# ipilter/RayTracerTest

Measured on AMD Instinct MI355X. Metric: Mray/s at 1920x1080x16spp, higher is better.
Workload: dtype f32

## Files before the change

raytracertest_amd/csrc/rt_kernels.hip:

```cpp
#include <stdlib.h>

#include "rt_dense.hpp"
#include "rt_query.hpp"
#include "rt_bvh.hpp"

namespace rtk {

template <bool FMA>
__global__ __launch_bounds__(256) void prep_triangles_kernel(const float4* __restrict__ verts, uint32_t n, bool edges,
                                                              float4* __restrict__ tri_a,
                                                              float* __restrict__ tri_b,
                                                              float4* __restrict__ color,
                                                              float4* __restrict__ normals) {
  const uint32_t i = blockIdx.x * 256u + threadIdx.x;
  if (i >= n) return;
  const float4 a = verts[3 * i + 0], b = verts[3 * i + 1], c = verts[3 * i + 2];
  const V3 v0 = {a.x, a.y, a.z};
  const V3 e1 = edges ? V3{b.x, b.y, b.z} : rtd::sub({b.x, b.y, b.z}, v0);
  const V3 e2 = edges ? V3{c.x, c.y, c.z} : rtd::sub({c.x, c.y, c.z}, v0);
  tri_a[2 * i + 0] = make_float4(e2.x, e2.y, e2.z, e1.x);
  tri_a[2 * i + 1] = make_float4(e1.y, e1.z, v0.x, v0.y);
  tri_b[i] = v0.z;
  const V3 nn = Math<FMA>::normalize(Math<FMA>::cross(e1, e2));
  color[i] = make_float4(rtd::absf(nn.x), rtd::absf(nn.y), rtd::absf(nn.z), 0.0f);
  if (normals != nullptr) {
    const V3 n0 = rtd::unpack_normal(a.w), n1 = rtd::unpack_normal(b.w), n2 = rtd::unpack_normal(c.w);
    normals[3 * i + 0] = make_float4(n0.x, n0.y, n0.z, 0.0f);
    normals[3 * i + 1] = make_float4(n1.x, n1.y, n1.z, 0.0f);
    normals[3 * i + 2] = make_float4(n2.x, n2.y, n2.z, 0.0f);
  }
}

__global__ __launch_bounds__(256) void convert_kernel(const float4* __restrict__ render,
                                                       const uint32_t* __restrict__ counts,
                                                       uint32_t* __restrict__ image, uint32_t npix) {
  const uint32_t i = blockIdx.x * 256u + threadIdx.x;
  if (i >= npix) return;
  const float4 s = render[i];
  const float cnt = static_cast<float>(counts[i]);
  image[i] = rtd::pack_color(255.0f * (s.x / cnt), 255.0f * (s.y / cnt), 255.0f * (s.z / cnt));
}

template <bool FMA>
__global__ void dbg_hit_triangle_kernel(uint32_t n, const float* __restrict__ rays,
                                        const float* __restrict__ tris, int eps_mode,
                                        int* __restrict__ hit, float* __restrict__ tuv,
                                        float* __restrict__ normal, float* __restrict__ point) {
  using M = Math<FMA>;
  const uint32_t i = blockIdx.x * blockDim.x + threadIdx.x;
  if (i >= n) return;
  const float* r = rays + 6 * static_cast<size_t>(i);
  const float* q = tris + 9 * static_cast<size_t>(i);
  const V3 o = {r[0], r[1], r[2]};
  const V3 d = M::normalize({r[3], r[4], r[5]});
  const V3 a = {q[0], q[1], q[2]}, b = {q[3], q[4], q[5]}, c = {q[6], q[7], q[8]};
  const V3 e1 = rtd::sub(b, a), e2 = rtd::sub(c, a);
  float t = 0.0f, u = 0.0f, v = 0.0f;
  int stage;
  const bool h = hit_triangle_exact<FMA>(o, d, a, e1, e2, eps_mode ? FLT_EPSILON : 0.0000000001f, t, u, v, stage);
  hit[i] = h ? 1 : 0;
  tuv[3 * i + 0] = t; tuv[3 * i + 1] = u; tuv[3 * i + 2] = v;
  const V3 nn = M::normalize(M::cross(e1, e2));
// ... 256 lines not shown
      case variant(P::Classify, 2): return launch_trace_kernel<F, 2, P::Classify>(p, filter, grid, lds, st);
      case variant(P::Classify, 4): return launch_trace_kernel<F, 4, P::Classify>(p, filter, grid, lds, st);
      case variant(P::ClassifyForms, 1): return launch_trace_kernel<F, 1, P::ClassifyForms>(p, filter, grid, lds, st);
      case variant(P::ClassifyForms, 2): return launch_trace_kernel<F, 2, P::ClassifyForms>(p, filter, grid, lds, st);
      case variant(P::ClassifyForms, 4): return launch_trace_kernel<F, 4, P::ClassifyForms>(p, filter, grid, lds, st);
      case variant(P::DenseLists, 1): return launch_trace_kernel<F, 1, P::DenseLists>(p, filter, grid, lds, st);
      case variant(P::DenseLists, 2): return launch_trace_kernel<F, 2, P::DenseLists>(p, filter, grid, lds, st);
      case variant(P::DenseLists, 4): return launch_trace_kernel<F, 4, P::DenseLists>(p, filter, grid, lds, st);
    }
  };
  if (fma) launch(std::true_type{}); else launch(std::false_type{});
  return hipGetLastError();
}

int trace_occupancy(int K, size_t lds) {
  int n = 0;
  hipError_t e;
  if (K == 1) e = hipOccupancyMaxActiveBlocksPerMultiprocessor(&n, trace_kernel<true, 1, true, false, TracePath::SmallLists>, 256, lds);
  else if (K == 2) e = hipOccupancyMaxActiveBlocksPerMultiprocessor(&n, trace_kernel<true, 2, true, false, TracePath::SmallLists>, 256, lds);
  else e = hipOccupancyMaxActiveBlocksPerMultiprocessor(&n, trace_kernel<true, 4, true, false, TracePath::Classify>, 256, lds);
  return e == hipSuccess ? n : -1;
}

hipError_t launch_convert(const float4* render, const uint32_t* counts, uint32_t* image, uint32_t npix,
                          hipStream_t st) {
  if (npix == 0) return hipSuccess;
  hipLaunchKernelGGL(convert_kernel, dim3(cdiv(npix, 256)), dim3(256), 0, st, render, counts, image, npix);
  return hipGetLastError();
}

hipError_t launch_dbg_hit_triangle(bool fma, uint32_t n, const float* rays, const float* tris, int eps_mode,
                                   int* hit, float* tuv, float* normal, float* point, hipStream_t st) {
  if (n == 0) return hipSuccess;
  if (fma) hipLaunchKernelGGL(dbg_hit_triangle_kernel<true>, dim3(cdiv(n, 64)), dim3(64), 0, st, n, rays, tris, eps_mode, hit, tuv, normal, point);
  else hipLaunchKernelGGL(dbg_hit_triangle_kernel<false>, dim3(cdiv(n, 64)), dim3(64), 0, st, n, rays, tris, eps_mode, hit, tuv, normal, point);
  return hipGetLastError();
}

hipError_t launch_super_bin(const TraceParams& p, bool fma, hipStream_t st) {
  if (p.super_lists == nullptr || p.macro_bounds == nullptr || p.macro_lists == nullptr || p.n_tris == 0u || p.rows == 0u || p.W == 0u || p.super_f == 0u ||
      p.super_chunks != cdiv(p.n_tris, kSuperChunk) || p.super_chunks > kSuperMaxChunks) return hipErrorInvalidValue;
  const dim3 mgrid(cdiv(p.W, p.macro_w), cdiv(p.rows, p.macro_h));
  const dim3 sgrid(p.super_nx * cdiv(mgrid.y, p.super_f), p.super_chunks);
  if (fma) {
    hipLaunchKernelGGL(macro_bounds_kernel<true>, mgrid, dim3(256), 0, st, p);
    hipLaunchKernelGGL(super_bin_kernel<true>, sgrid, dim3(256), 0, st, p);
  } else {
    hipLaunchKernelGGL(macro_bounds_kernel<false>, mgrid, dim3(256), 0, st, p);
    hipLaunchKernelGGL(super_bin_kernel<false>, sgrid, dim3(256), 0, st, p);
  }
// ... 160 lines not shown
```

raytracertest_amd/csrc/rt_kernels.hpp:

```cpp
#pragma once
#include <hip/hip_runtime.h>
#include <stdint.h>

namespace rtk {

constexpr uint32_t kSuperChunk = 1024u, kSuperMaxChunks = 64u;

struct TraceParams {
  float4*   render;
  uint32_t* counts;
  uint32_t* rng;
  uint32_t  W, H;
  uint32_t  row0, rows;
  uint32_t  npix;
  uint32_t  samples;
  float     cam[12];
  float     half_height, aspect, focal, aperture;
  float     tile_curv, tile_round;
  const float4* tri_a;
  const float*  tri_b;
  const float4* tri_color;
  uint32_t  n_tris;
  const float4* spheres;
  uint32_t  n_spheres;
  uint32_t  chunk;
  uint32_t  bin_list;
  uint32_t  block_list;
  unsigned long long* stats;
  uint32_t* image;
  const float4* tri_n;
#ifdef RT_TIMELINE
  unsigned long long* timeline;
#endif
  uint32_t* image_host;
// ... 15 lines not shown
};

constexpr uint32_t TRACE_ZERO_ACC = 1u;
constexpr uint32_t TRACE_EMIT_IMAGE = 2u;
constexpr uint32_t TRACE_NEAREST_HIT = 4u;
constexpr uint32_t TRACE_PRETEST = 32u;
constexpr uint32_t TRACE_NO_SURE_HIT = 64u;

enum class TracePath : uint32_t {
  FullScan,
  SmallLists,
  Classify,
  ClassifyForms,
  DenseLists,
};

hipError_t launch_rng_init(uint32_t* rng, uint32_t npix, uint32_t p0, const uint32_t seeded[6],
                           const uint32_t* jump, const uint32_t* win, hipStream_t st);
hipError_t launch_prep_triangles(bool fma, bool edges, const float4* verts, uint32_t n, float4* tri_a, float* tri_b,
                                 float4* color, float4* normals, hipStream_t st);
uint32_t trace_lds_bytes(const TraceParams& p, TracePath path);
hipError_t launch_trace(const TraceParams& p, bool fma, bool filter, TracePath path, int K, hipStream_t st);
int trace_occupancy(int K, size_t lds);
hipError_t launch_convert(const float4* render, const uint32_t* counts, uint32_t* image, uint32_t npix,
                          hipStream_t st);

uint32_t query_lds_bytes(uint32_t n_tris, int K);
hipError_t launch_query(const TraceParams& p, bool fma, int K, uint32_t n, const float* rays, const uint32_t* pixels,
                        float* rays_out, float4* hits, hipStream_t st);

#define RT_BVH_RHO 0.00390625f

struct BvhParams {
  const float4* nodes;
  const float4* records;
  uint32_t n_nodes;
  uint32_t n_leaf_records;
  uint32_t n_always;
  uint32_t stack_cap;
  float rho;
};
uint32_t query_bvh_lds_bytes(uint32_t stack_cap);
hipError_t launch_query_bvh(const TraceParams& p, const BvhParams& b, bool fma, uint32_t n, const float* rays, const uint32_t* pixels,
                            float* rays_out, float4* hits, hipStream_t st);

hipError_t launch_dbg_hit_triangle(bool fma, uint32_t n, const float* rays, const float* tris, int eps_mode,
                                   int* hit, float* tuv, float* normal, float* point, hipStream_t st);
bool trace_can_fuse(TracePath path, bool filter);
// ... 19 lines not shown
```

raytracertest_amd/csrc/rt_multi_api.hpp:

```cpp
#pragma once

namespace rtr {

bool env_on(const char* name) { const char* e = getenv(name); return e && e[0] == '1'; }

void multi_push_camera(rt_tracer* t) {
  Camera c;
  { std::lock_guard<std::mutex> lk(t->state_mu); c = t->cam; }
  for (rt_tracer* b : t->mg->bands) { std::lock_guard<std::mutex> lk(b->state_mu); b->cam = c; }
}

void multi_sync_all(rt_tracer* t) {
  MultiState& m = *t->mg;
  for (rt_tracer* b : m.bands) {
    b->use_device();
    b->sync_all();
  }
  m.group.sync();
}

void multi_frame_to_host(rt_tracer* t, int b) {
  MultiState& m = *t->mg;
  Group& g = m.group;
  HIP_CHECK(hipSetDevice(g.local[0].device));
// ... 367 lines not shown
    s += "]";
  }
  s += "}";
  return s;
}

void multi_read_buffer(rt_tracer* t, int which, void* dst, size_t bytes) {
  MultiState& m = *t->mg;
  Group& g = m.group;
  multi_sync_all(t);
  if (which == RT_BUF_IMAGE || which == RT_BUF_FRAME) {
    HIP_CHECK(hipSetDevice(g.local[0].device));
    HIP_CHECK(hipMemcpy(dst, g.d_frame[g.last_b < 0 ? 0 : g.last_b], bytes, hipMemcpyDeviceToHost));
    return;
  }
  const size_t per_px = which == RT_BUF_RENDER ? sizeof(float4) : sizeof(uint32_t);
  const size_t planes = which == RT_BUF_RNG ? 6u : 1u;
  const size_t frame_px = static_cast<size_t>(t->W) * t->H;
  if (bytes < frame_px * per_px * planes) throw HipFail{"rt_tracer_read_buffer: a multi-device tracer reads whole buffers only"};
  for (size_t k = 0; k < m.bands.size(); ++k) {
    rt_tracer* band = m.bands[k];
    band->use_device();
    const size_t band_px = band->npix(), off_px = static_cast<size_t>(g.bands[k].row0) * t->W;
    for (size_t p = 0; p < planes; ++p)
      HIP_CHECK(hipMemcpy(static_cast<char*>(dst) + (p * frame_px + off_px) * per_px,
                          static_cast<const char*>(buffer_ptr(band, which)) + p * band_px * per_px, band_px * per_px,
                          hipMemcpyDeviceToHost));
  }
}

void member_join(rt_tracer* t, uint32_t n_ranks, uint32_t rank, const uint8_t id[RT_GROUP_ID_BYTES], const uint32_t* begins) {
  if (t->grp) throw HipFail{"rt_tracer_join_group: already a member of a group"};
  uint32_t r0 = 0, rn = 0;
  if (begins) {
    if (begins[0] != 0u || begins[n_ranks] != t->H) throw HipFail{"rt_tracer_join_group_bands: the bands must cover rows 0 .. full_height"};
    for (uint32_t k = 0; k < n_ranks; ++k) if (begins[k + 1] <= begins[k]) throw HipFail{"rt_tracer_join_group_bands: empty or descending band"};
    r0 = begins[rank]; rn = begins[rank + 1] - begins[rank];
  } else {
    band_rows(t->H, n_ranks, rank, r0, rn);
  }
  if (!t->band_mode && n_ranks > 1u) throw HipFail{"rt_tracer_join_group: the tracer must own a row band (rt_options.full_height)"};
  if (r0 != t->row0 || rn != t->rows)
    throw HipFail{fmt("rt_tracer_join_group: rank %u of %u owns rows [%u, %u) of %u, the tracer has [%u, %u)", rank, n_ranks, r0,
                      r0 + rn, t->H, t->row0, t->row0 + t->rows)};
  Group* g = new Group();
  g->W = t->W; g->H = t->H;
// ... 50 lines not shown
```

raytracertest_amd/csrc/rt_rng_init.hip:

```cpp
#include "rt_device_math.hpp"
#include "rt_kernels.hpp"

namespace rtk {

using rtd::Rng;

static inline uint32_t cdiv(uint32_t a, uint32_t b) { return (a + b - 1) / b; }

constexpr uint32_t kRngWinEntries = 6u * 40u * 16u;
constexpr uint32_t kRngInitThreads = 512;

__device__ __forceinline__ uint32_t wave_xor(uint32_t v) {
#pragma unroll
  for (int off = 32; off >= 1; off >>= 1) v ^= static_cast<uint32_t>(__shfl_xor(static_cast<int>(v), off, 64));
  return v;
}

__global__ __launch_bounds__(kRngInitThreads, 4) void rng_init_kernel(uint32_t* __restrict__ rng, uint32_t npix,
                                                                    uint32_t p0, Rng seeded,
                                                                    const uint32_t* __restrict__ jump,
                                                                    const uint32_t* __restrict__ win) {
  extern __shared__ uint4 s_win[];
  uint32_t* const s_w4 = reinterpret_cast<uint32_t*>(s_win + kRngWinEntries);
  for (uint32_t i = threadIdx.x; i < kRngWinEntries; i += kRngInitThreads) {
// ... 55 lines not shown
    }
    uint32_t v[5] = {u[0], u[1], u[2], u[3], u[4]};
    for (uint32_t m = 0; m < 6u; ++m) {
      const uint4* __restrict__ T = s_win + m * 640u;
      const uint32_t* __restrict__ T4 = s_w4 + m * 640u;
      uint32_t r0 = 0u, r1 = 0u, r2 = 0u, r3 = 0u, r4 = 0u;
#pragma unroll 1
      for (uint32_t w = 0; w < 5u; ++w) {
        const uint32_t vw = w == 0u ? v[0] : w == 1u ? v[1] : w == 2u ? v[2] : w == 3u ? v[3] : v[4];
        const uint4* __restrict__ Tw = T + w * 128u;
        const uint32_t* __restrict__ T4w = T4 + w * 128u;
#pragma unroll
        for (uint32_t q = 0; q < 8u; ++q) {
          const uint32_t n = (vw >> (q * 4u)) & 15u;
          const uint4 e = Tw[q * 16u + n];
          r0 ^= e.x; r1 ^= e.y; r2 ^= e.z; r3 ^= e.w;
          r4 ^= T4w[q * 16u + n];
        }
      }
      if ((lane >> m) & 1u) { v[0] = r0; v[1] = r1; v[2] = r2; v[3] = r3; v[4] = r4; }
    }
    const uint32_t i = base + lane;
    if (i < npix) {
      rng[0 * static_cast<size_t>(npix) + i] = seeded.d;
      rng[1 * static_cast<size_t>(npix) + i] = v[0];
      rng[2 * static_cast<size_t>(npix) + i] = v[1];
      rng[3 * static_cast<size_t>(npix) + i] = v[2];
      rng[4 * static_cast<size_t>(npix) + i] = v[3];
      rng[5 * static_cast<size_t>(npix) + i] = v[4];
    }
  }
}

hipError_t launch_rng_init(uint32_t* rng, uint32_t npix, uint32_t p0, const uint32_t seeded[6],
                           const uint32_t* jump, const uint32_t* win, hipStream_t st) {
  Rng s = {seeded[0], seeded[1], seeded[2], seeded[3], seeded[4], seeded[5]};
  if (npix == 0) return hipSuccess;
  const uint32_t want = cdiv(npix, kRngInitThreads);
  uint32_t blocks = 1u;
  while (blocks < 512u && blocks * 2u <= want) blocks *= 2u;
  hipLaunchKernelGGL(rng_init_kernel, dim3(blocks), dim3(kRngInitThreads), kRngWinEntries * 20u, st, rng, npix, p0, s, jump, win);
  return hipGetLastError();
}

}
```

raytracertest_amd/csrc/rt_trace.hpp:

```cpp
#pragma once
#include "rt_lists.hpp"

namespace rtk {


template <bool FMA, int K, bool FILTER, bool STATS, class GetB>
__device__ __forceinline__ void test_triangle(const float4 A0, const float4 A1, GetB get_v0z, int tri_index,
                                              const V3 (&o)[K], const V3 (&d)[K], float (&best_t)[K],
                                              int (&best_i)[K], bool nearest, bool counted_lane, uint32_t valid_k,
                                              unsigned long long (&st_exit)[4],
                                              unsigned long long (&st_skip)[4]) {
  using M = Math<FMA>;
  const V3 e2 = {A0.x, A0.y, A0.z}, e1 = {A0.w, A1.x, A1.y};

  if constexpr (!FILTER) {
    const V3 v0 = {A1.z, A1.w, get_v0z()};
#pragma unroll
    for (int k = 0; k < K; ++k) {
      float t = 0.0f, u = 0.0f, v = 0.0f;
      int stage;
      const bool h = hit_triangle_exact<FMA>(o[k], d[k], v0, e1, e2, RT_EPS, t, u, v, stage);
      if (h && (nearest ? (t > 0.0f && t < best_t[k]) : best_t[k] < t)) {
        best_t[k] = t;
        best_i[k] = tri_index;
// ... 87 lines not shown
  const uint32_t cxp = inside ? px : 0u, cyp = inside ? ly : 0u;
  const size_t pix = static_cast<size_t>(cxp) + static_cast<size_t>(cyp) * p.W;

#ifdef RT_TIMELINE
  const size_t tl_slot = ((static_cast<size_t>(by) * gxb + bx) * 4u + wave) * 16u;
  auto tl_mark = [&](uint32_t i) {
    __builtin_amdgcn_sched_barrier(0);
    if (p.timeline != nullptr && lane == 0u) p.timeline[tl_slot + i] = __builtin_amdgcn_s_memrealtime();
    __builtin_amdgcn_sched_barrier(0);
  };
  if (p.timeline != nullptr && lane == 0u) {
    uint32_t hw, xcc;
    asm volatile("s_getreg_b32 %0, hwreg(HW_REG_HW_ID)" : "=s"(hw));
    asm volatile("s_getreg_b32 %0, hwreg(HW_REG_XCC_ID)" : "=s"(xcc));
    p.timeline[tl_slot + 6] = hw;
    p.timeline[tl_slot + 7] = (static_cast<unsigned long long>(xcc) << 32) | (__builtin_amdgcn_s_memrealtime() & 0xffffffffull);
  }
  tl_mark(0);
#else
  auto tl_mark = [](uint32_t) {};
#endif
  Rng rng;
  auto load_rng = [&] {
    rng.d = p.rng[0 * static_cast<size_t>(p.npix) + pix];
    rng.v0 = p.rng[1 * static_cast<size_t>(p.npix) + pix];
    rng.v1 = p.rng[2 * static_cast<size_t>(p.npix) + pix];
    rng.v2 = p.rng[3 * static_cast<size_t>(p.npix) + pix];
    rng.v3 = p.rng[4 * static_cast<size_t>(p.npix) + pix];
    rng.v4 = p.rng[5 * static_cast<size_t>(p.npix) + pix];
  };
  constexpr bool FORMS = Path == TracePath::ClassifyForms || Path == TracePath::DenseLists;
  constexpr bool RNG_LATE = FORMS;
  constexpr bool THIRD_BLOCK = true, THIRD_WAVE = !FORMS;
  if constexpr (!RNG_LATE) load_rng();


  const bool sure_ok = Path == TracePath::SmallLists && (p.flags & (TRACE_NEAREST_HIT | TRACE_NO_SURE_HIT)) == 0u && p.n_spheres == 0u && p.tri_n == nullptr;
  bool loaded_sure = false;
  uint32_t list_word = 0u;
  if constexpr (Path == TracePath::SmallLists) {
    if (p.tile_lists != nullptr) {
      const size_t slot0 = (static_cast<size_t>(by) * gxb + bx) * 4u + wave;
      list_word = static_cast<uint32_t>(__builtin_amdgcn_readfirstlane(static_cast<int>(p.tile_lists[slot0 * (1u + p.bin_list)])));
      loaded_sure = sure_ok && (list_word >> 31) != 0u;
    }
  }
  V3 po = {0.0f, 0.0f, 0.0f}, pd = {0.0f, 0.0f, 0.0f}, focal = {0.0f, 0.0f, 0.0f};
// ... 205 lines not shown
    __builtin_amdgcn_wave_barrier();
    list_count = count;
    if constexpr (STATS) { st_bin[0] += count; st_bin[1] += 1; }
    list_complete = true;
  }
  bool forms_ready = false;
  if constexpr (Path == TracePath::ClassifyForms) {
    const uint32_t next0 = classify(0u, std::true_type{});
    list_complete = next0 >= src_count;
    forms_ready = pretest && list_complete;
  }
  if constexpr (Path == TracePath::DenseLists) forms_ready = true;
  if constexpr (RNG_LATE) load_rng();
  tl_mark(1);
  float4 sure_col = make_float4(0.0f, 0.0f, 0.0f, 0.0f);
  const bool sure_sums = Path == TracePath::SmallLists && p.sure_table != nullptr;
  if constexpr (Path == TracePath::SmallLists) { if (sure_hit_tile) sure_col = sure_sums ? p.sure_table[sure_winner] : p.tri_color[sure_winner]; }
  if constexpr (STATS && Path == TracePath::SmallLists) {
    if (lane == 0u && p.stats != nullptr)
      atomicAdd(p.stats + (sure_hit_tile ? 13 : list_count == 0u ? 11 : list_count == 1u ? 12 : list_count == 2u ? 14 : 15), 1ull);
  }
  const uint32_t iters = FUSE ? p.iters : 1u;
  float rx = 0.0f, ry = 0.0f, rz = 0.0f, rw = 0.0f;
  uint32_t cnt_first = 0u;
  for (uint32_t it = 0; it < iters; ++it) {
  if constexpr (FUSE) { ax = 0.0f; ay = 0.0f; az = 0.0f; }
  uint32_t traced_samples = p.samples;
  if constexpr (Path == TracePath::SmallLists) {
    if (sure_hit_tile) {
      rtd::rng_discard(rng, 3u * p.samples);
      if (sure_sums) { ax = sure_col.x; ay = sure_col.y; az = sure_col.z; }
      else for (uint32_t s = 0; s < p.samples; ++s) { ax += sure_col.x; ay += sure_col.y; az += sure_col.z; }
      if constexpr (STATS) st_pre += (p.samples + static_cast<uint32_t>(K) - 1u) / static_cast<uint32_t>(K);
      traced_samples = 0u;
    }
  }
  for (uint32_t s0 = 0; s0 < traced_samples; s0 += K) {
    if (s0 == static_cast<uint32_t>(K)) tl_mark(2);
    const uint32_t valid_k = (p.samples - s0 < static_cast<uint32_t>(K)) ? p.samples - s0 : static_cast<uint32_t>(K);
    V3 o[K], d[K];
    float best_t[K];
    int best_i[K];
#pragma unroll
    for (int k = 0; k < K; ++k) {
      if (static_cast<uint32_t>(k) < valid_k) get_ray<FMA>(p, focal, rng, o[k], d[k]);
      else { o[k] = {0.0f, 0.0f, 0.0f}; d[k] = {0.0f, 0.0f, -1.0f}; }
      best_t[k] = nearest ? FLT_MAX : -FLT_MAX;
// ... 147 lines not shown
            const V3 nn = M::normalize(rtd::sub(hp, {sph.x, sph.y, sph.z}));
            r = rtd::absf(nn.x); g = rtd::absf(nn.y); b = rtd::absf(nn.z);
          }
        } else {
          if constexpr (FMA) {
            r = __builtin_fmaf(d[k].x, 0.2f, 0.15f * 0.8f);
            g = __builtin_fmaf(d[k].y, 0.2f, 0.11f * 0.8f);
            b = __builtin_fmaf(d[k].z, 0.2f, 0.13f * 0.8f);
          } else {
            r = 0.15f * 0.8f + d[k].x * 0.2f;
            g = 0.11f * 0.8f + d[k].y * 0.2f;
            b = 0.13f * 0.8f + d[k].z * 0.2f;
          }
        }
        ax += r; ay += g; az += b;
      }
    }
  }

  if constexpr (FUSE) {
    if (it == 0u && !(p.flags & TRACE_ZERO_ACC) && inside) {
      const float4 r0 = p.render[pix];
      rx = r0.x; ry = r0.y; rz = r0.z; rw = r0.w;
      cnt_first = p.counts[pix];
    }
    rx += ax; ry += ay; rz += az;
  }
  }
  tl_mark(3);
  uint32_t pix_lo = static_cast<uint32_t>(pix);
  asm volatile("" : "+v"(pix_lo));
  const size_t pix_e = pix_lo;
  if (inside) {
    float4 acc_in = make_float4(0.0f, 0.0f, 0.0f, 0.0f);
    uint32_t cnt_in = 0u;
    if constexpr (!FUSE) {
      if (!(p.flags & TRACE_ZERO_ACC)) {
        acc_in = p.render[pix_e];
        cnt_in = p.counts[pix_e];
      }
    }
    const uint32_t cnt = FUSE ? cnt_first + iters * p.samples : cnt_in + p.samples;
    p.counts[pix_e] = cnt;
    float4 acc = acc_in;
    if constexpr (FUSE) {
      acc = make_float4(rx, ry, rz, rw);
    } else {
      acc.x += ax; acc.y += ay; acc.z += az;
    }
    p.render[pix_e] = acc;
    if (p.flags & TRACE_EMIT_IMAGE) {
      const float c = static_cast<float>(cnt);
      uint32_t bgra;
      if (!FUSE && sure_sums && sure_hit_tile && (p.flags & TRACE_ZERO_ACC)) bgra = __builtin_bit_cast(uint32_t, sure_col.w);
      else bgra = rtd::pack_color(255.0f * (acc.x / c), 255.0f * (acc.y / c), 255.0f * (acc.z / c));
      p.image[pix_e] = bgra;
      if (p.image_host != nullptr) p.image_host[pix_e] = bgra;
    }
    p.rng[0 * static_cast<size_t>(p.npix) + pix_e] = rng.d;
    p.rng[1 * static_cast<size_t>(p.npix) + pix_e] = rng.v0;
    p.rng[2 * static_cast<size_t>(p.npix) + pix_e] = rng.v1;
    p.rng[3 * static_cast<size_t>(p.npix) + pix_e] = rng.v2;
    p.rng[4 * static_cast<size_t>(p.npix) + pix_e] = rng.v3;
    p.rng[5 * static_cast<size_t>(p.npix) + pix_e] = rng.v4;
  }
  tl_mark(4);
  if constexpr (STATS) {
    if (lane == 0 && p.stats != nullptr) {
#pragma unroll
      for (int e = 0; e < 4; ++e) {
        atomicAdd(p.stats + e, st_exit[e]);
        atomicAdd(p.stats + 4 + e, st_skip[e]);
      }
      atomicAdd(p.stats + 8, st_bin[0]);
      atomicAdd(p.stats + 9, st_bin[1]);
      atomicAdd(p.stats + 10, st_pre);
    }
  }
}


}
// ... 1 lines not shown
```

raytracertest_amd/csrc/rt_tracer.hip:

```cpp
#include "rt_tracer.hpp"

#include <map>

namespace rtr {

std::mutex g_err_mu;
std::string g_last_error;

void set_global_error(const std::string& s) {
  std::lock_guard<std::mutex> lk(g_err_mu);
  g_last_error = s;
  static const bool log = getenv("RT_MI355X_LOG") != nullptr;
  if (log) fprintf(stderr, "[rt_mi355x] %s\n", s.c_str());
}

std::mutex g_jump_mu;
std::vector<uint32_t> g_jump_host;
std::map<int, uint32_t*> g_jump_dev;

const std::vector<uint32_t>& jump_host() {
  std::lock_guard<std::mutex> lk(g_jump_mu);
  if (g_jump_host.empty()) g_jump_host = rth::build_jump_table();
  return g_jump_host;
}
// ... 484 lines not shown
    t->launch_instrumented(p, samples);
    HIP_CHECK(hipMemcpy(out, counters.get(), 16 * sizeof(uint64_t), hipMemcpyDeviceToHost));
  });
}

int rt_tracer_sync(rt_tracer* t) {
  if (!t) return RT_ERR_INVALID;
  if (t->mg) return guarded(t, [&] { multi_sync_all(t); });
  return guarded(t, [&] {
    t->use_device();
    t->sync_all();
    if (t->grp) t->grp->sync();
  });
}

int rt_tracer_kernel_time(rt_tracer* t, double* total_ms, uint64_t* launches, int reset_after) {
  return read_clock(t, false, total_ms, launches, reset_after);
}
int rt_tracer_launch_time(rt_tracer* t, double* total_ms, uint64_t* launches, int reset_after) {
  return read_clock(t, true, total_ms, launches, reset_after);
}

size_t rt_tracer_buffer_bytes(rt_tracer* t, int which) { return t ? buffer_bytes(t, which) : 0; }
void* rt_tracer_device_pointer(rt_tracer* t, int which) { return t ? buffer_ptr(t, which) : nullptr; }

int rt_tracer_read_buffer(rt_tracer* t, int which, void* dst, size_t bytes) {
  if (!t || !dst) return RT_ERR_INVALID;
  if (t->mg) {
    if (bytes > buffer_bytes(t, which) || buffer_bytes(t, which) == 0) return RT_ERR_INVALID;
    return guarded(t, [&] { multi_read_buffer(t, which, dst, bytes); });
  }
  if (buffer_ptr(t, which) == nullptr || bytes > buffer_bytes(t, which)) return RT_ERR_INVALID;
  return guarded(t, [&] {
    t->use_device();
    HIP_CHECK(hipStreamSynchronize(t->main_stream()));
    if (t->grp) t->grp->sync();
    HIP_CHECK(hipMemcpy(dst, buffer_ptr(t, which), bytes, hipMemcpyDeviceToHost));
  });
}

int rt_tracer_copy_buffer_to_device(rt_tracer* t, int which, void* dst_device, size_t bytes) {
  if (!t || !dst_device || buffer_ptr(t, which) == nullptr || bytes > buffer_bytes(t, which)) return RT_ERR_INVALID;
  if (t->mg) return guarded(t, [&] {
    multi_sync_all(t);
    HIP_CHECK(hipSetDevice(t->mg->group.local[0].device));
    HIP_CHECK(hipMemcpy(dst_device, buffer_ptr(t, which), bytes, hipMemcpyDeviceToDevice));
  });
  return guarded(t, [&] {
    t->use_device();
    if (t->grp && which == RT_BUF_FRAME) t->grp->sync();
    HIP_CHECK(hipMemcpyAsync(dst_device, buffer_ptr(t, which), bytes, hipMemcpyDeviceToDevice, t->main_stream()));
    HIP_CHECK(hipStreamSynchronize(t->main_stream()));
  });
}

int rt_tracer_copy_buffer_to_device_async(rt_tracer* t, int which, void* dst_device, size_t bytes) {
  if (!t || !dst_device || buffer_ptr(t, which) == nullptr || bytes > buffer_bytes(t, which)) return RT_ERR_INVALID;
  if (t->mg || which == RT_BUF_FRAME) { t->set_error("rt_tracer_copy_buffer_to_device_async: per-stream copies are for plain tracers' own buffers"); return RT_ERR_STATE; }
  return guarded(t, [&] {
    t->use_device();
    HIP_CHECK(hipMemcpyAsync(dst_device, buffer_ptr(t, which), bytes, hipMemcpyDeviceToDevice, t->main_stream()));
  });
}

void* rt_tracer_stream(rt_tracer* t) { return (t && !t->mg) ? static_cast<void*>(t->stream) : nullptr; }
void* rt_tracer_stream_b(rt_tracer* t) { return (t && !t->mg) ? static_cast<void*>(t->stream_b) : nullptr; }

int rt_tracer_info(rt_tracer* t, uint32_t out[8]) {
  if (!t || !out) return RT_ERR_INVALID;
  if (t->mg) {
    (void)rt_tracer_info(t->mg->bands[0], out);
    out[3] = (t->W + 31) / 32; out[4] = (t->H + 7) / 8;
    out[7] = static_cast<uint32_t>(t->device);
    return RT_OK;
  }
  out[0] = t->last_k; out[1] = t->last_chunk; out[2] = t->last_lds;
  out[3] = (t->W + 31) / 32; out[4] = (t->rows + 7) / 8;
  out[5] = t->n_tris; out[6] = t->n_spheres; out[7] = static_cast<uint32_t>(t->device);
  return RT_OK;
}


int rt_tracer_create_multi(const uint32_t imageSize[2], const float cameraPosition[3], const float cameraAngles[2],
// ... 123 lines not shown
```

raytracertest_amd/csrc/rt_tracer.hpp:

```cpp
#pragma once
#include <algorithm>
#include <atomic>
#include <chrono>
#include <condition_variable>
#include <functional>
#include <cmath>
#include <cstdio>
#include <cstring>
#include <ctime>
#include <mutex>
#include <optional>
#include <string>
#include <thread>
#include <vector>

#include "../../include/rt_mi355x.h"
#include "rt_device_math.hpp"
#include "rt_hip_host.hpp"
#include "rt_kernels.hpp"
#include "rt_rng_host.hpp"

namespace rtr {

struct Env {
// ... 315 lines not shown

struct rt_tracer {
  rtr::Group* grp = nullptr;
  rtr::MultiState* mg = nullptr;
  rtr::Env env;
  int device = 0;
  uint32_t W = 0, H = 0;
  uint32_t row0 = 0, rows = 0;
  bool band_mode = false;
  uint64_t seed = 1;
  bool fma = true, filter = true, bin = true, nearest_hit = false;
  bool smooth_normals = false;
  uint32_t k_req = 0, chunk_req = 0, bin_list_req = 0;

  rtr::Stream stream;
  rtr::Stream stream_b;
  rtr::Stream stream_l;
  rtr::Stream stream_q;
  rtr::Event join_event, fork_event;
  bool b_dirty = false;
  bool a_dirty = false;
  bool split_launches = true;

  std::mutex order_mu;
  hipStream_t main_stream() {
    std::lock_guard<std::mutex> lk(order_mu);
    if (b_dirty) {
      HIP_CHECK(hipEventRecord(join_event, stream_b));
      HIP_CHECK(hipStreamWaitEvent(stream, join_event, 0));
      b_dirty = false;
    }
    a_dirty = true;
    return stream;
  }
  void fork_b() {
    std::lock_guard<std::mutex> lk(order_mu);
    if (!a_dirty) return;
    HIP_CHECK(hipEventRecord(fork_event, stream));
    HIP_CHECK(hipStreamWaitEvent(stream_b, fork_event, 0));
    a_dirty = false;
  }
  void mark_b_dirty() { std::lock_guard<std::mutex> lk(order_mu); b_dirty = true; }
  rtr::DevArray<float4> d_render;
  rtr::DevArray<uint32_t> d_counts, d_image, d_rng;
  rtr::PinnedArray<uint32_t> h_image;
  rtr::PinnedArray<uint32_t> h_image_alt;
  uint32_t* image_mirror = nullptr;
  rtr::Event handoff_event;
  int handoff_next = 0;
  rtr::DevArray<float4> d_tri;
  rtr::DevArray<float> d_tri_b;
  rtr::DevArray<float4> d_tri_color;
  rtr::DevArray<float4> d_tri_n;
  uint32_t n_tris = 0;
  rtr::DevArray<float4> d_spheres;
  uint32_t n_spheres = 0;
  rtr::DevArray<float> d_q_rays;
  rtr::DevArray<uint32_t> d_q_pixels;
  rtr::DevArray<float4> d_q_hits;
  rtr::Event query_done;
  void wait_queries() { if (query_done) HIP_CHECK(hipEventSynchronize(query_done)); }
  uint32_t query_accel = RT_QUERY_SCAN;
  uint32_t query_slack_milli = 1000u;
  rtr::DevArray<float4> d_bvh_nodes, d_bvh_records;
  bool bvh_built = false;
  uint32_t bvh_scene = 0;
  uint64_t bvh_info[6] = {0, 0, 0, 0, 0, 0};
// ... 28 lines not shown
      stopped = true;
      render.wait_idle();
      stopped = false;
    }
  }

  void release_buffers() {
    d_render.reset(); d_counts.reset(); d_image.reset(); d_rng.reset(); h_image.reset(); h_image_alt.reset();
  }

  void quiesce() {
    (void)hipSetDevice(device);
    for (const rtr::Stream* s : {&stream_b, &stream, &stream_l, &stream_q}) if (*s) (void)hipStreamSynchronize(*s);
    if (query_done) (void)hipEventSynchronize(query_done);
    clock.drain();
  }

  void create_states() {
    uint32_t seeded[6];
    rth::seed_state(seed, seeded);
    const uint32_t p0 = row0 * W;
    if (static_cast<uint64_t>(W) * H > 0xFFFFFFFFull) throw rtr::HipFail{"frames above 2^32 pixels are not supported (32-bit pixel index, Kernels.cuh:128)"};
    uint32_t* const tables = rtr::jump_device(device);
    HIP_CHECK(rtk::launch_rng_init(d_rng.get(), npix(), p0, seeded, tables, tables + rtr::kJumpWords, main_stream()));
  }

  void create_buffers() {
    const size_t n = npix();
    if (n == 0) throw rtr::HipFail{"image has no pixels"};
    d_rng.ensure(n * 6); d_render.ensure(n); d_counts.ensure(n); d_image.ensure(n); h_image.ensure(n); h_image_alt.ensure(n);
    memset(h_image.get(), 0, n * sizeof(uint32_t));
    memset(h_image_alt.get(), 0, n * sizeof(uint32_t));
    HIP_CHECK(hipMemsetAsync(d_render.get(), 0, n * sizeof(float4), main_stream()));
    HIP_CHECK(hipMemsetAsync(d_counts.get(), 0, n * sizeof(uint32_t), main_stream()));
    HIP_CHECK(hipMemsetAsync(d_image.get(), 0, n * sizeof(uint32_t), main_stream()));
    create_states();
    HIP_CHECK(hipStreamSynchronize(main_stream()));
  }

  void reshape(uint32_t w, uint32_t h, uint32_t r0, uint32_t n) {
    HIP_CHECK(hipStreamSynchronize(main_stream()));
    sync_list_stream();
    release_buffers();
    W = w; H = h; row0 = r0; rows = n;
    lists.key.reset();
    create_buffers();
  }

  void copy_image_to(uint32_t* target) {
    HIP_CHECK(hipMemcpyAsync(target, d_image.get(), static_cast<size_t>(npix()) * sizeof(uint32_t), hipMemcpyDeviceToDevice, main_stream()));
  }

  void tile_corner_bound(rtk::TraceParams& p) const {
    p.tile_curv = -1.0f; p.tile_round = 0.0f;
    double G[3][3];
    for (int i = 0; i < 3; ++i)
      for (int j = 0; j < 3; ++j) {
        G[i][j] = 0.0;
// ... 6 lines not shown
      lmin = std::min(lmin, G[i][i] - off);
    }
    if (!(lmin > 0.25) || !(lmax < 4.0)) return;
    const double hh = std::fabs(static_cast<double>(p.half_height)), asp = std::fabs(static_cast<double>(p.aspect));
    const double a = 7.0 * 2.0 * hh * asp / static_cast<double>(W), b = 7.0 * 2.0 * hh / static_cast<double>(H);
    if (!(0.5 * (a * a + b * b) * (lmax / lmin) <= 0.1 * std::min(a, b))) return;
    const double foc = std::fabs(static_cast<double>(p.focal));
#ifndef RT_TILE_CURV_SCALE
#define RT_TILE_CURV_SCALE 1.0
#endif
    const double curv = foc * 0.5 * (a * a + b * b) * (lmax / lmin) * 1.001 * RT_TILE_CURV_SCALE + 1e-30;
    const double pos = std::max(std::fabs(p.cam[9]), std::max(std::fabs(p.cam[10]), std::fabs(p.cam[11])));
    const double round = foc * (1.0 + hh * asp + hh) + pos;
    if (!(curv <= 1e30) || !(round <= 1e30)) return;
    p.tile_curv = std::nextafter(static_cast<float>(curv), 3.0e38f);
    p.tile_round = std::nextafter(static_cast<float>(round), 3.0e38f);
  }

  rtk::TraceParams params(uint32_t samples) {
    rtk::TraceParams p;
    memset(&p, 0, sizeof p);
    rtr::Camera c;
    { std::lock_guard<std::mutex> lk(state_mu); c = cam; }
    p.render = d_render.get(); p.counts = d_counts.get(); p.rng = d_rng.get();
    p.W = W; p.H = H; p.row0 = row0; p.rows = rows; p.npix = npix(); p.samples = samples;
    for (int col = 0; col < 4; ++col)
      for (int r = 0; r < 3; ++r) p.cam[col * 3 + r] = c.M[col * 4 + r];
    p.half_height = c.tan_half_fov();
    p.aspect = static_cast<float>(W) / static_cast<float>(H);
    p.focal = c.focal; p.aperture = c.aperture;
    tile_corner_bound(p);
    p.tri_a = d_tri.get(); p.tri_b = d_tri_b.get(); p.tri_color = d_tri_color.get(); p.n_tris = n_tris;
    p.tri_n = smooth_normals ? d_tri_n.get() : nullptr;
    p.stats = nullptr;
    p.spheres = d_spheres.get(); p.n_spheres = n_spheres;
    p.chunk = chunk_req ? chunk_req : 1024u;
    if (p.chunk > 4096u) p.chunk = 4096u;
    uint32_t want = bin_list_req ? bin_list_req : ((n_tris + 31u) / 32u) * 32u;
    want = ((want + 31u) / 32u) * 32u;
    p.bin_list = want < 32u ? 32u : want > (bin_list_req ? 960u : 256u) ? (bin_list_req ? 960u : 256u) : want;
    p.block_list = n_tris > p.bin_list ? 1024u : 0u;
    if (p.block_list != 0u && !bin_list_req) p.bin_list = 192u;
    if (pretest && filter && bin && n_tris >= kPretestMinTris && n_tris <= 50000u) {
      p.pretest_on = 1u;
      if (!bin_list_req) p.bin_list = RT_PRETEST_LIST;
      else p.bin_list = (p.bin_list + 1u) & ~1u;
      if (p.block_list != 0u) p.block_list = 448u;
// ... 9 lines not shown
  int pick_k(uint32_t samples) const {
    if (k_req == 1 || k_req == 2 || k_req == 4) return static_cast<int>(k_req);
    const uint32_t want = (n_tris <= 128u) ? 2u : 4u;
    return samples >= want ? static_cast<int>(want) : samples >= 2 ? 2 : 1;
  }

  void enqueue_trace_launch(uint32_t samples, uint32_t flags, int sync_after, uint32_t iters = 1,
                            uint32_t* host_image = nullptr, bool allow_split = true) {
    const int K = pick_k(samples);
    rtk::TraceParams p = params(samples);
    p.iters = iters;
    p.image_host = host_image;
    p.flags = flags | mode_flags(p);
    p.image = d_image.get();
    const rtk::TracePath path = trace_path(p);
    bool have_lists = false;
    const bool build_lists = prepare_tile_lists(p, path, (flags & rtk::TRACE_ZERO_ACC) != 0u, have_lists);
    attach_sure_table(p, have_lists);
    last_k = K; last_chunk = p.chunk;
    last_lds = rtk::trace_lds_bytes(p, path == rtk::TracePath::DenseLists ? rtk::TracePath::ClassifyForms : path);
    const uint32_t r0 = allow_split ? split_row(p.rows) : 0u;
    rtr::EventPair e;
    const bool timed = clock.start(sync_after == 1, r0 != 0u, e);
    if (r0 == 0u) {
      (void)main_stream();
      if (build_lists) build_tile_lists_ahead(p);
      lists.attach(p, row0, have_lists);
      if (timed) HIP_CHECK(hipEventRecord(e.a, stream));
      if (have_lists) lists.wait(stream, 0);
      attach_macro_lists(p, path, 0, stream, (flags & rtk::TRACE_ZERO_ACC) != 0u);
      HIP_CHECK(rtk::launch_trace(p, fma, filter, path, K, stream));
      if (timed) HIP_CHECK(hipEventRecord(e.b, stream));
    } else {
      fork_b();
      if (build_lists) build_tile_lists_ahead(p);
      const bool stagger = stagger_next.exchange(false);
      const bool interleave = have_lists && want_interleave();
      if (have_lists && interleave != rows_interleaved) {
        (void)main_stream();
        fork_b();
        rows_interleaved = interleave;
        if (env.log) fprintf(stderr, "[rt_mi355x] split launches: halves by %s\n", interleave ? "even / odd block rows" : "rows");
      }
      rtk::TraceParams half[2] = {sub_band(p, 0u, r0), sub_band(p, r0, p.rows - r0)};
      if (interleave) { half[0] = p; half[1] = p; half[0].row_il = half[1].row_il = 1u; half[1].row_phase = 1u; }
      hipStream_t st[2] = {stream, stream_b};
      if (timed) HIP_CHECK(hipEventRecord(e.a, stream));
      for (int h = 0; h < 2; ++h) {
        lists.attach(half[h], row0, have_lists);
        if (have_lists) lists.wait(st[h], h);
        if (h == 1 && stagger) {
          const uint32_t us = static_cast<uint32_t>(clock.last_half_ms() * 450.0f);
          if (us >= 5u) HIP_CHECK(rtk::launch_delay(us, stream_b));
          else HIP_CHECK(hipStreamWaitEvent(stream_b, stagger_event, 0));
        }
        const rtk::TracePath half_path = trace_path(half[h]);
        attach_macro_lists(half[h], half_path, h, st[h], (flags & rtk::TRACE_ZERO_ACC) != 0u);
        HIP_CHECK(rtk::launch_trace(half[h], fma, filter, half_path, K, st[h]));
        if (h == 0 && stagger) HIP_CHECK(hipEventRecord(stagger_event, stream));
      }
      if (timed) { HIP_CHECK(hipEventRecord(e.b, stream)); HIP_CHECK(hipEventRecord(e.c, stream_b)); }
      mark_b_dirty();
    }
    if (timed) clock.enqueued(std::move(e), sync_after);
  }

  static rtk::TraceParams sub_band(const rtk::TraceParams& p, uint32_t off, uint32_t n) {
    rtk::TraceParams q = p;
    const size_t px = static_cast<size_t>(off) * p.W;
    q.row0 = p.row0 + off; q.rows = n;
    q.render = p.render + px; q.counts = p.counts + px; q.rng = p.rng + px;
    q.image = p.image + px;
    if (p.image_host != nullptr) q.image_host = p.image_host + px;
    return q;
  }

  void clear_accumulators() {
    HIP_CHECK(hipMemsetAsync(d_render.get(), 0, static_cast<size_t>(npix()) * sizeof(float4), main_stream()));
    HIP_CHECK(hipMemsetAsync(d_counts.get(), 0, static_cast<size_t>(npix()) * sizeof(uint32_t), main_stream()));
  }

  void convert() {
    HIP_CHECK(rtk::launch_convert(d_render.get(), d_counts.get(), d_image.get(), npix(), main_stream()));
  }

  static void sync_polling(hipStream_t st) {
    const auto t0 = std::chrono::steady_clock::now();
    for (;;) {
      const hipError_t e = hipStreamQuery(st);
      if (e == hipSuccess) return;
      if (e != hipErrorNotReady) HIP_CHECK(e);
      if (std::chrono::steady_clock::now() - t0 > std::chrono::milliseconds(2)) break;
    }
    (void)hipGetLastError();
    HIP_CHECK(hipStreamSynchronize(st));
  }

  void fetch_image() {
    HIP_CHECK(hipMemcpyAsync(h_image.get(), d_image.get(), static_cast<size_t>(npix()) * sizeof(uint32_t),
                             hipMemcpyDeviceToHost, main_stream()));
    HIP_CHECK(hipStreamSynchronize(main_stream()));
  }

  rtr::TileListRing lists;
  rtr::Event stagger_event;
  std::atomic<bool> stagger_next{true};
// ... 57 lines not shown
    }
    p.sure_table = d_sure_table.get();
  }

  void build_tile_lists_ahead(const rtk::TraceParams& p_band) {
    const uint64_t m = lists.build_ahead();
    rtk::TraceParams q = p_band;
    lists.attach(q, row0, true);
    const uint32_t sr = split_row(rows);
    if (sr != 0u && d_half_cost.get() != nullptr && env.row_interleave < 0 && (m % 32u) == 0u) { q.half_cost = d_half_cost.get(); q.cost_split_brow = sr / 8u; }
    HIP_CHECK(rtk::launch_tile_lists(q, fma, stream_l));
    lists.built();
    if (q.half_cost != nullptr) HIP_CHECK(rtk::launch_publish_half_cost(d_half_cost.get(), h_half_cost.get(), stream_l));
  }

  void launch_instrumented(rtk::TraceParams& p, uint32_t samples) {
    const rtk::TracePath path = trace_path(p);
    bool have_lists = false;
    (void)prepare_tile_lists(p, path, true, have_lists);
    sync_list_stream();
    lists.attach(p, row0, have_lists);
    if (have_lists) HIP_CHECK(rtk::launch_tile_lists(p, fma, main_stream()));
    attach_macro_lists(p, path, 0, main_stream());
    HIP_CHECK(rtk::launch_trace(p, fma, filter, path, pick_k(samples), main_stream()));
    HIP_CHECK(hipStreamSynchronize(main_stream()));
  }

  rtr::HalfLists half_lists[2];
  bool macro = true;
  bool pretest = true;
  bool sure_hit = true;
  bool reuse_across_traces = true;
  static constexpr uint32_t kPretestMinTris = 4096;
  static constexpr uint32_t kMacroW = 128, kMacroH = 64, kMacroCapMax = 65536;
#ifndef RT_SUPER_F
#define RT_SUPER_F 4
#endif
  static constexpr uint32_t kSuperF = RT_SUPER_F, kSuperMinTris = 2048;
  bool super_level = true;

  void attach_macro_lists(rtk::TraceParams& p, rtk::TracePath path, int half, hipStream_t st, bool first_launch_of_trace = true) {
    p.macro_lists = nullptr;
    if (!macro || path == rtk::TracePath::FullScan || path == rtk::TracePath::SmallLists) return;
    rtr::HalfLists& h = half_lists[half];
    p.macro_w = kMacroW; p.macro_h = kMacroH;
    p.macro_nx = (p.W + p.macro_w - 1u) / p.macro_w;
    const uint32_t ny = (p.rows + p.macro_h - 1u) / p.macro_h;
// ... 165 lines not shown
```

Before: 580,100.

## Make per-pixel sample count and Weyl RNG state uniform host-side scalars

Every pixel holds the same sample count and the same Weyl sequence value, so both are now kept as host-tracked scalars passed in the kernel parameters instead of per-pixel device arrays. The trace kernel no longer reads or writes the counts plane or the Weyl RNG plane, which cuts global memory traffic per pixel. The device planes are filled lazily with a memset only when a caller reads those buffers. This relies on counts and Weyl state being uniform across pixels and adds locking to keep the host state consistent across streams.

```diff
diff --git a/raytracertest_amd/csrc/rt_kernels.hip b/raytracertest_amd/csrc/rt_kernels.hip
--- a/raytracertest_amd/csrc/rt_kernels.hip
+++ b/raytracertest_amd/csrc/rt_kernels.hip
@@ -32,12 +32,12 @@
 }
 
 __global__ __launch_bounds__(256) void convert_kernel(const float4* __restrict__ render,
-                                                       const uint32_t* __restrict__ counts,
+                                                       uint32_t count,
                                                        uint32_t* __restrict__ image, uint32_t npix) {
   const uint32_t i = blockIdx.x * 256u + threadIdx.x;
   if (i >= npix) return;
   const float4 s = render[i];
-  const float cnt = static_cast<float>(counts[i]);
+  const float cnt = static_cast<float>(count);
   image[i] = rtd::pack_color(255.0f * (s.x / cnt), 255.0f * (s.y / cnt), 255.0f * (s.z / cnt));
 }
 
@@ -340,10 +340,9 @@
   return e == hipSuccess ? n : -1;
 }
 
-hipError_t launch_convert(const float4* render, const uint32_t* counts, uint32_t* image, uint32_t npix,
-                          hipStream_t st) {
+hipError_t launch_convert(const float4* render, uint32_t count, uint32_t* image, uint32_t npix, hipStream_t st) {
   if (npix == 0) return hipSuccess;
-  hipLaunchKernelGGL(convert_kernel, dim3(cdiv(npix, 256)), dim3(256), 0, st, render, counts, image, npix);
+  hipLaunchKernelGGL(convert_kernel, dim3(cdiv(npix, 256)), dim3(256), 0, st, render, count, image, npix);
   return hipGetLastError();
 }
 
diff --git a/raytracertest_amd/csrc/rt_kernels.hpp b/raytracertest_amd/csrc/rt_kernels.hpp
--- a/raytracertest_amd/csrc/rt_kernels.hpp
+++ b/raytracertest_amd/csrc/rt_kernels.hpp
@@ -8,8 +8,8 @@
 
 struct TraceParams {
   float4*   render;
-  uint32_t* counts;
   uint32_t* rng;
+  uint32_t  weyl, count;
   uint32_t  W, H;
   uint32_t  row0, rows;
   uint32_t  npix;
@@ -71,8 +71,7 @@
 uint32_t trace_lds_bytes(const TraceParams& p, TracePath path);
 hipError_t launch_trace(const TraceParams& p, bool fma, bool filter, TracePath path, int K, hipStream_t st);
 int trace_occupancy(int K, size_t lds);
-hipError_t launch_convert(const float4* render, const uint32_t* counts, uint32_t* image, uint32_t npix,
-                          hipStream_t st);
+hipError_t launch_convert(const float4* render, uint32_t count, uint32_t* image, uint32_t npix, hipStream_t st);
 
 uint32_t query_lds_bytes(uint32_t n_tris, int K);
 hipError_t launch_query(const TraceParams& p, bool fma, int K, uint32_t n, const float* rays, const uint32_t* pixels,
diff --git a/raytracertest_amd/csrc/rt_multi_api.hpp b/raytracertest_amd/csrc/rt_multi_api.hpp
--- a/raytracertest_amd/csrc/rt_multi_api.hpp
+++ b/raytracertest_amd/csrc/rt_multi_api.hpp
@@ -413,6 +413,8 @@
     rt_tracer* band = m.bands[k];
     band->use_device();
     const size_t band_px = band->npix(), off_px = static_cast<size_t>(g.bands[k].row0) * t->W;
+    band->materialise(which);
+    HIP_CHECK(hipStreamSynchronize(band->main_stream()));
     for (size_t p = 0; p < planes; ++p)
       HIP_CHECK(hipMemcpy(static_cast<char*>(dst) + (p * frame_px + off_px) * per_px,
                           static_cast<const char*>(buffer_ptr(band, which)) + p * band_px * per_px, band_px * per_px,
diff --git a/raytracertest_amd/csrc/rt_rng_init.hip b/raytracertest_amd/csrc/rt_rng_init.hip
--- a/raytracertest_amd/csrc/rt_rng_init.hip
+++ b/raytracertest_amd/csrc/rt_rng_init.hip
@@ -101,7 +101,6 @@
     }
     const uint32_t i = base + lane;
     if (i < npix) {
-      rng[0 * static_cast<size_t>(npix) + i] = seeded.d;
       rng[1 * static_cast<size_t>(npix) + i] = v[0];
       rng[2 * static_cast<size_t>(npix) + i] = v[1];
       rng[3 * static_cast<size_t>(npix) + i] = v[2];
diff --git a/raytracertest_amd/csrc/rt_trace.hpp b/raytracertest_amd/csrc/rt_trace.hpp
--- a/raytracertest_amd/csrc/rt_trace.hpp
+++ b/raytracertest_amd/csrc/rt_trace.hpp
@@ -133,7 +133,7 @@
 #endif
   Rng rng;
   auto load_rng = [&] {
-    rng.d = p.rng[0 * static_cast<size_t>(p.npix) + pix];
+    rng.d = p.weyl;
     rng.v0 = p.rng[1 * static_cast<size_t>(p.npix) + pix];
     rng.v1 = p.rng[2 * static_cast<size_t>(p.npix) + pix];
     rng.v2 = p.rng[3 * static_cast<size_t>(p.npix) + pix];
@@ -385,7 +385,6 @@
   }
   const uint32_t iters = FUSE ? p.iters : 1u;
   float rx = 0.0f, ry = 0.0f, rz = 0.0f, rw = 0.0f;
-  uint32_t cnt_first = 0u;
   for (uint32_t it = 0; it < iters; ++it) {
   if constexpr (FUSE) { ax = 0.0f; ay = 0.0f; az = 0.0f; }
   uint32_t traced_samples = p.samples;
@@ -579,7 +578,6 @@
     if (it == 0u && !(p.flags & TRACE_ZERO_ACC) && inside) {
       const float4 r0 = p.render[pix];
       rx = r0.x; ry = r0.y; rz = r0.z; rw = r0.w;
-      cnt_first = p.counts[pix];
     }
     rx += ax; ry += ay; rz += az;
   }
@@ -590,15 +588,10 @@
   const size_t pix_e = pix_lo;
   if (inside) {
     float4 acc_in = make_float4(0.0f, 0.0f, 0.0f, 0.0f);
-    uint32_t cnt_in = 0u;
     if constexpr (!FUSE) {
-      if (!(p.flags & TRACE_ZERO_ACC)) {
-        acc_in = p.render[pix_e];
-        cnt_in = p.counts[pix_e];
-      }
-    }
-    const uint32_t cnt = FUSE ? cnt_first + iters * p.samples : cnt_in + p.samples;
-    p.counts[pix_e] = cnt;
+      if (!(p.flags & TRACE_ZERO_ACC)) acc_in = p.render[pix_e];
+    }
+    const uint32_t cnt = p.count + iters * p.samples;
     float4 acc = acc_in;
     if constexpr (FUSE) {
       acc = make_float4(rx, ry, rz, rw);
@@ -614,7 +607,6 @@
       p.image[pix_e] = bgra;
       if (p.image_host != nullptr) p.image_host[pix_e] = bgra;
     }
-    p.rng[0 * static_cast<size_t>(p.npix) + pix_e] = rng.d;
     p.rng[1 * static_cast<size_t>(p.npix) + pix_e] = rng.v0;
     p.rng[2 * static_cast<size_t>(p.npix) + pix_e] = rng.v1;
     p.rng[3 * static_cast<size_t>(p.npix) + pix_e] = rng.v2;
diff --git a/raytracertest_amd/csrc/rt_tracer.hip b/raytracertest_amd/csrc/rt_tracer.hip
--- a/raytracertest_amd/csrc/rt_tracer.hip
+++ b/raytracertest_amd/csrc/rt_tracer.hip
@@ -530,7 +530,12 @@
 }
 
 size_t rt_tracer_buffer_bytes(rt_tracer* t, int which) { return t ? buffer_bytes(t, which) : 0; }
-void* rt_tracer_device_pointer(rt_tracer* t, int which) { return t ? buffer_ptr(t, which) : nullptr; }
+void* rt_tracer_device_pointer(rt_tracer* t, int which) {
+  if (!t) return nullptr;
+  if (!t->mg && (which == RT_BUF_RNG || which == RT_BUF_COUNTS) &&
+      guarded(t, [&] { t->use_device(); t->materialise(which); }) != RT_OK) return nullptr;
+  return buffer_ptr(t, which);
+}
 
 int rt_tracer_read_buffer(rt_tracer* t, int which, void* dst, size_t bytes) {
   if (!t || !dst) return RT_ERR_INVALID;
@@ -541,6 +546,7 @@
   if (buffer_ptr(t, which) == nullptr || bytes > buffer_bytes(t, which)) return RT_ERR_INVALID;
   return guarded(t, [&] {
     t->use_device();
+    t->materialise(which);
     HIP_CHECK(hipStreamSynchronize(t->main_stream()));
     if (t->grp) t->grp->sync();
     HIP_CHECK(hipMemcpy(dst, buffer_ptr(t, which), bytes, hipMemcpyDeviceToHost));
@@ -557,6 +563,7 @@
   return guarded(t, [&] {
     t->use_device();
     if (t->grp && which == RT_BUF_FRAME) t->grp->sync();
+    t->materialise(which);
     HIP_CHECK(hipMemcpyAsync(dst_device, buffer_ptr(t, which), bytes, hipMemcpyDeviceToDevice, t->main_stream()));
     HIP_CHECK(hipStreamSynchronize(t->main_stream()));
   });
@@ -567,6 +574,7 @@
   if (t->mg || which == RT_BUF_FRAME) { t->set_error("rt_tracer_copy_buffer_to_device_async: per-stream copies are for plain tracers' own buffers"); return RT_ERR_STATE; }
   return guarded(t, [&] {
     t->use_device();
+    t->materialise(which);
     HIP_CHECK(hipMemcpyAsync(dst_device, buffer_ptr(t, which), bytes, hipMemcpyDeviceToDevice, t->main_stream()));
   });
 }
diff --git a/raytracertest_amd/csrc/rt_tracer.hpp b/raytracertest_amd/csrc/rt_tracer.hpp
--- a/raytracertest_amd/csrc/rt_tracer.hpp
+++ b/raytracertest_amd/csrc/rt_tracer.hpp
@@ -361,9 +361,9 @@
   bool a_dirty = false;
   bool split_launches = true;
 
-  std::mutex order_mu;
+  std::recursive_mutex order_mu;
   hipStream_t main_stream() {
-    std::lock_guard<std::mutex> lk(order_mu);
+    std::lock_guard<std::recursive_mutex> lk(order_mu);
     if (b_dirty) {
       HIP_CHECK(hipEventRecord(join_event, stream_b));
       HIP_CHECK(hipStreamWaitEvent(stream, join_event, 0));
@@ -373,15 +373,36 @@
     return stream;
   }
   void fork_b() {
-    std::lock_guard<std::mutex> lk(order_mu);
+    std::lock_guard<std::recursive_mutex> lk(order_mu);
     if (!a_dirty) return;
     HIP_CHECK(hipEventRecord(fork_event, stream));
     HIP_CHECK(hipStreamWaitEvent(stream_b, fork_event, 0));
     a_dirty = false;
   }
-  void mark_b_dirty() { std::lock_guard<std::mutex> lk(order_mu); b_dirty = true; }
+  void mark_b_dirty() { std::lock_guard<std::recursive_mutex> lk(order_mu); b_dirty = true; }
   rtr::DevArray<float4> d_render;
   rtr::DevArray<uint32_t> d_counts, d_image, d_rng;
+  uint32_t weyl_now = 0, count_now = 0;
+  uint32_t weyl_plane = 0, count_plane = 0;
+  bool weyl_plane_ok = false, count_plane_ok = false;
+  void take_uniform_state(rtk::TraceParams& p) {
+    if (p.flags & rtk::TRACE_ZERO_ACC) count_now = 0u;
+    p.weyl = weyl_now; p.count = count_now;
+    const uint32_t done = p.samples * (p.iters > 1u ? p.iters : 1u);
+    weyl_now += 362437u * 3u * done;
+    count_now += done;
+  }
+  void materialise(int which) {
+    std::lock_guard<std::recursive_mutex> lk(order_mu);
+    if (which == RT_BUF_RNG && !(weyl_plane_ok && weyl_plane == weyl_now) && d_rng.get() != nullptr) {
+      HIP_CHECK(hipMemsetD32Async(reinterpret_cast<hipDeviceptr_t>(d_rng.get()), static_cast<int>(weyl_now), npix(), main_stream()));
+      weyl_plane = weyl_now; weyl_plane_ok = true;
+    }
+    if (which == RT_BUF_COUNTS && !(count_plane_ok && count_plane == count_now) && d_counts.get() != nullptr) {
+      HIP_CHECK(hipMemsetD32Async(reinterpret_cast<hipDeviceptr_t>(d_counts.get()), static_cast<int>(count_now), npix(), main_stream()));
+      count_plane = count_now; count_plane_ok = true;
+    }
+  }
   rtr::PinnedArray<uint32_t> h_image;
   rtr::PinnedArray<uint32_t> h_image_alt;
   uint32_t* image_mirror = nullptr;
@@ -456,7 +477,9 @@
     const uint32_t p0 = row0 * W;
     if (static_cast<uint64_t>(W) * H > 0xFFFFFFFFull) throw rtr::HipFail{"frames above 2^32 pixels are not supported (32-bit pixel index, Kernels.cuh:128)"};
     uint32_t* const tables = rtr::jump_device(device);
+    std::lock_guard<std::recursive_mutex> lk(order_mu);
     HIP_CHECK(rtk::launch_rng_init(d_rng.get(), npix(), p0, seeded, tables, tables + rtr::kJumpWords, main_stream()));
+    weyl_now = seeded[0]; weyl_plane_ok = false;
   }
 
   void create_buffers() {
@@ -466,8 +489,8 @@
     memset(h_image.get(), 0, n * sizeof(uint32_t));
     memset(h_image_alt.get(), 0, n * sizeof(uint32_t));
     HIP_CHECK(hipMemsetAsync(d_render.get(), 0, n * sizeof(float4), main_stream()));
-    HIP_CHECK(hipMemsetAsync(d_counts.get(), 0, n * sizeof(uint32_t), main_stream()));
     HIP_CHECK(hipMemsetAsync(d_image.get(), 0, n * sizeof(uint32_t), main_stream()));
+    { std::lock_guard<std::recursive_mutex> lk(order_mu); count_now = 0u; count_plane_ok = false; }
     create_states();
     HIP_CHECK(hipStreamSynchronize(main_stream()));
   }
@@ -520,7 +543,7 @@
     memset(&p, 0, sizeof p);
     rtr::Camera c;
     { std::lock_guard<std::mutex> lk(state_mu); c = cam; }
-    p.render = d_render.get(); p.counts = d_counts.get(); p.rng = d_rng.get();
+    p.render = d_render.get(); p.rng = d_rng.get();
     p.W = W; p.H = H; p.row0 = row0; p.rows = rows; p.npix = npix(); p.samples = samples;
     for (int col = 0; col < 4; ++col)
       for (int r = 0; r < 3; ++r) p.cam[col * 3 + r] = c.M[col * 4 + r];
@@ -576,6 +599,8 @@
     const uint32_t r0 = allow_split ? split_row(p.rows) : 0u;
     rtr::EventPair e;
     const bool timed = clock.start(sync_after == 1, r0 != 0u, e);
+    std::unique_lock<std::recursive_mutex> uniform_lk(order_mu);
+    take_uniform_state(p);
     if (r0 == 0u) {
       (void)main_stream();
       if (build_lists) build_tile_lists_ahead(p);
@@ -616,6 +641,7 @@
       if (timed) { HIP_CHECK(hipEventRecord(e.b, stream)); HIP_CHECK(hipEventRecord(e.c, stream_b)); }
       mark_b_dirty();
     }
+    uniform_lk.unlock();
     if (timed) clock.enqueued(std::move(e), sync_after);
   }
 
@@ -623,19 +649,21 @@
     rtk::TraceParams q = p;
     const size_t px = static_cast<size_t>(off) * p.W;
     q.row0 = p.row0 + off; q.rows = n;
-    q.render = p.render + px; q.counts = p.counts + px; q.rng = p.rng + px;
+    q.render = p.render + px; q.rng = p.rng + px;
     q.image = p.image + px;
     if (p.image_host != nullptr) q.image_host = p.image_host + px;
     return q;
   }
 
   void clear_accumulators() {
+    std::lock_guard<std::recursive_mutex> lk(order_mu);
     HIP_CHECK(hipMemsetAsync(d_render.get(), 0, static_cast<size_t>(npix()) * sizeof(float4), main_stream()));
-    HIP_CHECK(hipMemsetAsync(d_counts.get(), 0, static_cast<size_t>(npix()) * sizeof(uint32_t), main_stream()));
+    count_now = 0u;
   }
 
   void convert() {
-    HIP_CHECK(rtk::launch_convert(d_render.get(), d_counts.get(), d_image.get(), npix(), main_stream()));
+    std::lock_guard<std::recursive_mutex> lk(order_mu);
+    HIP_CHECK(rtk::launch_convert(d_render.get(), count_now, d_image.get(), npix(), main_stream()));
   }
 
   static void sync_polling(hipStream_t st) {
@@ -739,7 +767,11 @@
     lists.attach(p, row0, have_lists);
     if (have_lists) HIP_CHECK(rtk::launch_tile_lists(p, fma, main_stream()));
     attach_macro_lists(p, path, 0, main_stream());
-    HIP_CHECK(rtk::launch_trace(p, fma, filter, path, pick_k(samples), main_stream()));
+    {
+      std::lock_guard<std::recursive_mutex> lk(order_mu);
+      take_uniform_state(p);
+      HIP_CHECK(rtk::launch_trace(p, fma, filter, path, pick_k(samples), main_stream()));
+    }
     HIP_CHECK(hipStreamSynchronize(main_stream()));
   }
 
```

Result: faster. 596,200 (median of 6 runs) (+2.8%).
